# dimforge/salva

Hardware: AMD Instinct MI355X
Metric: particle-steps/sec (3D DFSPH) (higher is better)
Workload: dtype f32

## Files before the change

salva_amd/csrc/pairs.h:

```cpp
#pragma once
#include <cstdlib>

#include "tile.h"

namespace salva {

struct RecPW { float4 p, w; };
struct RecPK { float4 p; float k; };

__device__ __forceinline__ float rho0_of(const StepCtx& c, uint32_t model) {
    return (c.nmodels == 1) ? c.rho0_single : c.rho0_tab[model];
}

template <uint32_t DS>
__device__ __forceinline__ uint32_t pw_dist(const StepCtx& c, const Tile& t) { return DS ? DS * 16u : (t.stage_cap(c) + t.SB) * 16u; }
template <uint32_t DS>
__device__ __forceinline__ uint32_t pk_dist(const StepCtx& c, const Tile& t) { return DS ? DS * 16u : (t.stage_cap(c) + 2u * t.SB) * 16u; }

__device__ __forceinline__ RecPW load_pw(uint32_t o, uint32_t dist) {
    RecPW r{lds_ld16(o), lds_ld16(o + dist)};
    asm volatile("" ::"v"(r.w.w));
    return r;
}
__device__ __forceinline__ RecPK load_pk(uint32_t o, uint32_t dist) { return RecPK{lds_ld16(o), lds_ld4((o >> 2) + dist)}; }
// ... 215 lines not shown
        else if ((DSV) == FIXED_DS_LARGE) SALVA_LAUNCH_TILE_3(kernel<FIXED_DS_LARGE>, kernel<FIXED_DS_SMALL>, FIXED_DS_SMALL, kernel<0u>, c, L, lds, s, __VA_ARGS__); \
        else SALVA_LAUNCH_TILE_3(kernel<0u>, kernel<FIXED_DS_SMALL>, FIXED_DS_SMALL, kernel<0u>, c, L, lds, s, __VA_ARGS__); \
    } while (0)
static inline uint32_t pick_ds(uint32_t slots_needed, uint32_t level) {
    const uint32_t ds[3] = {FIXED_DS_SMALL, FIXED_DS_LARGE, 0u};
    uint32_t k = slots_needed <= FIXED_DS_SMALL ? 0u : (slots_needed <= FIXED_DS_LARGE ? 1u : 2u);
    k += level;
    return ds[k < 2u ? k : 2u];
}
static inline uint32_t pw_slots(const TileLds& L) { return L.sum_slots(); }
static inline uint32_t pw_bytes(const TileLds& L, uint32_t ds, bool errtab) {
    return (ds ? 2u * ds : 2u * pw_slots(L)) * 16u + (errtab ? TILE_ERR_BYTES : 0u) + 32u;
}
static inline uint32_t pick_ds_p3(uint32_t s, uint32_t level) {
    const uint32_t ds[4] = {P3_DS_THREE, P3_DS_TWO, P3_DS_ONE, 0u};
    uint32_t k = s <= P3_DS_THREE ? 0u : (s <= P3_DS_TWO ? 1u : (s <= P3_DS_ONE ? 2u : 3u));
    k += level;
    return ds[k < 3u ? k : 3u];
}
static inline uint32_t p3_bytes(const TileLds& L, uint32_t ds, uint32_t nmodels, bool with_bv) {
    const uint32_t dist8 = ds ? ds * 8u : ((L.max_halo_fluid * 8u + 15u) & ~15u);
    const uint32_t bb = with_bv ? 32u : 16u;
    const uint32_t by_maxima = ((L.max_halo_fluid * 8u + 15u) & ~15u) + bb * L.max_halo_boundary;
    const uint32_t by_raw = ((L.raw_slots() * 8u + 15u) & ~15u) + (bb - 8u) * L.max_halo_boundary;
    static const uint32_t pad = getenv("SALVA_HIP_P3_PAD") ? (uint32_t)atoi(getenv("SALVA_HIP_P3_PAD")) : 0u;
    return 2u * dist8 + (by_raw < by_maxima ? by_raw : by_maxima) + ((TILE_MAX_WAVES * nmodels * 4u + 15u) & ~15u) + 32u + pad;
}
static inline uint32_t pick_ds_p2(uint32_t n, uint32_t level) {
    const uint32_t ds[4] = {P2_DS_THREE, P3_DS_TWO, P3_DS_ONE, 0u};
    uint32_t k = n <= P2_DS_THREE ? 0u : (n <= P3_DS_TWO ? 1u : (n <= P3_DS_ONE ? 2u : 3u));
    k += level;
    return ds[k < 3u ? k : 3u];
}
#define SALVA_LAUNCH_P3(kernel, DSV, c, L, lds, s, ...)                                                                                          \
    do {                                                                                                                                         \
        if ((DSV) == P3_DS_THREE) SALVA_LAUNCH_TILE_3(kernel<P3_DS_THREE>, kernel<P3_DS_THREE>, P3_DS_THREE, kernel<0u>, c, L, lds, s, __VA_ARGS__); \
        else if ((DSV) == P3_DS_TWO) SALVA_LAUNCH_TILE_3(kernel<P3_DS_TWO>, kernel<P3_DS_THREE>, P3_DS_THREE, kernel<0u>, c, L, lds, s, __VA_ARGS__); \
        else if ((DSV) == P3_DS_ONE) SALVA_LAUNCH_TILE_3(kernel<P3_DS_ONE>, kernel<P3_DS_THREE>, P3_DS_THREE, kernel<0u>, c, L, lds, s, __VA_ARGS__); \
        else SALVA_LAUNCH_TILE_3(kernel<0u>, kernel<P3_DS_THREE>, P3_DS_THREE, kernel<0u>, c, L, lds, s, __VA_ARGS__);                             \
    } while (0)
#define SALVA_LAUNCH_P2(kernel, DSV, c, L, lds, s, ...)                                                                                          \
    do {                                                                                                                                         \
        if ((DSV) == P2_DS_THREE) SALVA_LAUNCH_TILE_3(kernel<P2_DS_THREE>, kernel<P2_DS_THREE>, P2_DS_THREE, kernel<0u>, c, L, lds, s, __VA_ARGS__); \
        else if ((DSV) == P3_DS_TWO) SALVA_LAUNCH_TILE_3(kernel<P3_DS_TWO>, kernel<P2_DS_THREE>, P2_DS_THREE, kernel<0u>, c, L, lds, s, __VA_ARGS__); \
        else if ((DSV) == P3_DS_ONE) SALVA_LAUNCH_TILE_3(kernel<P3_DS_ONE>, kernel<P2_DS_THREE>, P2_DS_THREE, kernel<0u>, c, L, lds, s, __VA_ARGS__); \
        else SALVA_LAUNCH_TILE_3(kernel<0u>, kernel<P2_DS_THREE>, P2_DS_THREE, kernel<0u>, c, L, lds, s, __VA_ARGS__);                             \
    } while (0)
static inline uint32_t pk_slots(const TileLds& L) { return L.sum_slots() + L.max_halo_boundary; }
static inline uint32_t pk_bytes(const TileLds& L, uint32_t ds) {
    return (ds ? ds : pk_slots(L)) * 16u + ((L.max_halo_fluid + 63u) & ~63u) * 4u + 32u;
}


}
```

salva_amd/csrc/switches.h:

```cpp
#pragma once
#include <cstdint>

namespace salva {

struct Switches {
    bool spec_off = true;
    bool spec_tight = false;
    bool defer_off = false;
    bool spec_apply_off = false;
    bool spec_dist_off = false;
    bool overlap_exchange = true;
    bool chain_off = false;
    bool pre_off = false;
    bool no_publish = false;
    bool split_off = false;
    uint32_t split_forced = 0;
    bool classes_off = false, classes_forced = false, light_on = false;
    bool ref_off = false, ref_forced = false;
    bool ref_tight = false;
    bool compact_halo = false;
    bool no_planes = false;
    bool no_fused_div = false;
    bool two_mass_off = false;
    uint32_t max_masses = 2;
    bool fold_off = false;
    uint32_t fold_forced = 0;
    int sort_mode = -1;
    uint32_t ds_level = 0;
    bool trust_cap0 = false;
    uint32_t list_cap0 = 0;
    bool dcs_batch_off = false;
    uint32_t dcsb_cap0 = 0;
    int field_arm = 0;
    bool tile_trace = false;
    bool dist_trace = false;
#ifdef SALVA_HIP_DIAG
    int sched_mode = 0;
    bool tile_threads_set = false;
    uint32_t tile_threads = 0;
    bool no_pipeline = false;
    uint32_t pipe_waves = 0;
    bool tile_timing = false;
#endif
    static Switches from_env();
};

}
```

salva_amd/csrc/tile.h:

```cpp
#pragma once
#include "common.h"
#include "device_types.h"

namespace salva {

#ifndef SALVA_TX
#define SALVA_TX 4
#endif
constexpr int TX = SALVA_TX, TY = 4, TZ = 4;
constexpr int TCELLS = TX * TY * TZ;
constexpr int HX = TX + 2, HY = TY + 2, HZ = TZ + 2;
constexpr int HCELLS = HX * HY * HZ;
constexpr int TILE_MAX_WAVES = 12;
constexpr int TILE_MAX_THREADS = TILE_MAX_WAVES * WAVE;

__host__ __device__ inline int floor_div(int a, int b) { return (a >= 0) ? a / b : -((-a + b - 1) / b); }

__host__ __device__ inline uint32_t ellq(uint32_t q) { return (q >> 2) * (4u * (uint32_t)WAVE) + (q & 3u); }

constexpr uint32_t TILE_TABLE_BYTES = 4 * (2 * (HCELLS + 1) + 2 * HCELLS) + 16;

struct TileLds {
    uint32_t max_halo_fluid = 0, max_halo_boundary = 0, threads = 4 * WAVE;
    uint32_t max_sum = 0;
    uint32_t max_raw = 0;
    uint32_t ds_level = 0;
    uint32_t raw_slots() const { return max_raw ? max_raw : max_halo_fluid + max_halo_boundary; }
    uint32_t sum_slots() const {
        const uint32_t worst = ((max_halo_fluid + 63u) & ~63u) + max_halo_boundary;
        return max_sum ? (max_sum < worst ? max_sum : worst) : worst;
    }
    uint32_t bytes(uint32_t bytes_per_fluid_slot, uint32_t bytes_per_boundary_slot, uint32_t narrays,
                   bool with_cell_tables = false) const {
        const uint32_t separate = ((max_halo_fluid + 63u) & ~63u) * bytes_per_fluid_slot + max_halo_boundary * bytes_per_boundary_slot;
        const uint32_t wide = bytes_per_fluid_slot > bytes_per_boundary_slot ? bytes_per_fluid_slot : bytes_per_boundary_slot;
        const uint32_t joint = sum_slots() * wide;
        return (with_cell_tables ? TILE_TABLE_BYTES : 0u) + (joint < separate ? joint : separate) + 16u * narrays;
    }
};

#ifndef SALVA_FIXED_DS_SMALL
#define SALVA_FIXED_DS_SMALL 2448
#endif
constexpr uint32_t FIXED_DS_SMALL = SALVA_FIXED_DS_SMALL, FIXED_DS_LARGE = 3984;
#ifndef SALVA_P3_DS3
#define SALVA_P3_DS3 2080
#endif
constexpr uint32_t P3_DS_THREE = SALVA_P3_DS3, P3_DS_TWO = 3360, P3_DS_ONE = 4064;
#ifndef SALVA_P2_DS3
#define SALVA_P2_DS3 2464
#endif
constexpr uint32_t P2_DS_THREE = SALVA_P2_DS3;
static_assert((P3_DS_THREE % 64 == 32 && P3_DS_TWO % 64 == 32 && P3_DS_ONE % 64 == 32 && P2_DS_THREE % 64 == 32) || SALVA_P3_DS3 != 2080 || SALVA_P2_DS3 != 2464,
              "plane distances: odd multiples of 256 bytes");
constexpr uint32_t TILE_PART_SHIFT = 28;
constexpr uint32_t TILE_PART_WHOLE = (uint32_t)(TX - 1) << 2;
// ... 943 lines not shown
```

salva_amd/csrc/world.h:

```cpp
#pragma once
#include <functional>
#include <string>
#include <map>
#include <memory>
#include <vector>

#include "../../include/salva_hip.h"
#include "common.h"
#include "device_types.h"
#include "comm.h"
#include "dist.h"
#include "kernels.h"
#include "elastic.h"
#include "switches.h"
#include "mesh.h"
#include "compound.h"
#include "sink.h"
#include "field.h"
#include "anisotropy.h"
#include "surface.h"
#include "fluidcast.h"

namespace salva {

// ... 407 lines not shown
        GridShape gs;
        double dcs_ms = 0.0;
        int attempt = 0;
        bool dcs_undo = false;
        uint32_t split_s_cur = 0;
        bool two_mass = false;
        uint32_t nmass = 0; float mass_classes[4] = {0.0f, 0.0f, 0.0f, 0.0f}; uint64_t mass_cmask = 0;
        size_t dist_ev_used = 0; std::vector<std::pair<size_t, int>> dist_ev_pairs;
    } pass;
    struct GridTabs;
    struct PassSnapshot;
    void prepare_working_set(SalvaHipStepStats& st);
    GridShape choose_grid();
    void ensure_slot_tables(uint32_t nslots_bound);
    bool run_pass(const PassSnapshot& snap, float& dt, const float g[3], SalvaHipStepStats& st);
    void enqueue_grid_keys(GridTabs& T, const GridShape& gs, bool counting, bool mass, const uint32_t* gate);
    void enqueue_grid_sort(GridTabs& T, const GridShape& gs, bool counting, const uint32_t* gate);
    size_t tile_scan_temp(const GridShape& gs);
    uint32_t enqueue_grid_tiles(GridTabs& T, const GridShape& gs, StepCtx c, size_t tb, const uint32_t* gate, bool publish);
    bool predict_totals(const GridShape& gs, TileAcc& tt) const;
    void reorder_working_set(bool timers);
    void size_pass(uint32_t seq_totals);
    void fill_tile_tables(bool again);
    void build_lists();
    void density_and_solve(StepCtx& c, float& dt, const float g[3], SalvaHipStepStats& st, bool timers);
    void publish_end_of_step(const PassSnapshot& snap);
    void adopt_chain_outcome(StepCtx& c, float& dt, const float g[3], SalvaHipStepStats& st, bool timers);
    int finish_substep(float dt, SalvaHipStepStats& st);
    void record_timers(SalvaHipStepStats& st);
    void raise_step_flags();
    bool has_force(int kind) const;
    bool counting_sort_for(size_t ncf, uint32_t np) const;
    void grow_list_caps(uint32_t need_ff, uint32_t need_fb);
    int cfl_mode = 0;
    float cfl_coeff = 0.4f;
    int cfl_min_sub = 1, cfl_max_sub = 10;
    float step_total = 0.0f, step_remaining = 0.0f;
    std::vector<float> substeps;
    float choose_substep(const StepCtx& c);
    FluidArrays arrays(int which);
    DistArrays dist_arrays(int which);
    void dist_prepare();
    void dist_build_lists();
    template <typename T, typename Gather, typename Scatter> void refresh_ghosts(T* field, Gather gather, Scatter scatter);
    void refresh_f32(float* field);
    void refresh_f4(float4* field);
    void ensure_particle_capacity(size_t cap);
    void allreduce_host_u64(std::vector<unsigned long long>& v);
    uint32_t num_models() const { return (uint32_t)std::max<size_t>(fluids.size(), 1); }
    template <typename Decide> void allreduced_test(const SolveCtl* record, Decide&& decide);
    void finalize_solve(SolveCtl* ctl, SolveCtl* pub, uint32_t skipped);
    void finalize_solve_ring(int it, SolveCtl* pub);

    const Switches sw = Switches::from_env();
    uint32_t last_iters[NUM_SOLVES] = {1u, 1u, 1u};
    uint32_t prev_iters[NUM_SOLVES] = {1u, 1u, 1u};
    float mass_uniform = 0.0f;
    bool mass_known = false;
    bool flags_clean = false;
    bool lists_checked = false;
    uint32_t fold_relax = 0;
    bool fold_locked = false;
    bool split_on = false;
    int32_t bbox_used_last[6] = {0, 0, 0, 0, 0, 0}; bool bbox_used_valid = false;
    TileAcc pred_tt{};
    uint32_t pred_n = 0; bool pred_valid = false;
    bool ref_pred_valid = false;
    uint32_t ref_pred[3] = {0, 0, 0}, ref_pred_n = 0;
    bool ref_last = false;
    RefCaps ref_last_caps{0xffffffffu, 0xffffffffu, 0xffffffffu};
    TileLds lds_full;
    uint32_t ref_last_nslots_bound = 0;
    struct Tallies { uint64_t chain_steps = 0, chain_breaks = 0, spec_misses = 0, ref_passes = 0, ref_misses = 0, pre_adopted = 0, pre_dropped = 0; } tally;

    hipStream_t stream = nullptr;
    hipStream_t stream2 = nullptr;
    hipStream_t dl_stream = nullptr;
    hipEvent_t ev_dl_ready = nullptr, ev_dl_done = nullptr;
    DevBuf<float> dl_dev[2];
    float* h_dl[2] = {nullptr, nullptr};
    size_t h_dl_cap[2] = {0, 0};
    struct PendingDownload { bool active = false; float* dst[2] = {nullptr, nullptr}; bool staged[2] = {false, false}; size_t bytes = 0; } dl;
    hipEvent_t ev_pre_refresh = nullptr, ev_interior = nullptr;
    hipEvent_t ev_spec_eval = nullptr, ev_spec_apply = nullptr;
    template <typename Launch> void evaluate_split(const StepCtx& c, int iteration, Launch&& launch);
    uint32_t n = 0, nb = 0;

    DevBuf<float4> st_pos, st_vel, st_dv, st_acc;
    DevBuf<uint32_t> st_model;
    bool staging_current = true, sorted_valid = false, acc_user = false;

    DevBuf<float4> posm[2], vel[2], dv[2];
    DevBuf<uint32_t> model[2], perm[2];
// ... 136 lines not shown
```

salva_amd/csrc/world.hip:

```cpp
#include "world.h"
#include "bbox.h"

#include <algorithm>
#include <cmath>
#include <cstring>
#include <limits>

#include <mutex>
#include <unordered_map>

namespace salva {

void raise_tile_lds_limit(const void* kernel, uint32_t bytes) {
    if (bytes > 160u * 1024u)
        throw HipError(SALVA_HIP_E_CAPACITY, "a tile's halo does not fit the 160 KiB LDS (particles are compressed far beyond rest density)");
    static std::mutex mu;
    static std::unordered_map<const void*, uint32_t> granted;
    std::lock_guard<std::mutex> lock(mu);
    uint32_t& g = granted[kernel];
    if (bytes <= g) return;
    const uint32_t want = std::min<uint32_t>(160u * 1024u, std::max<uint32_t>(bytes + bytes / 4, 64u * 1024u));
    SALVA_HIP_CHECK(hipFuncSetAttribute(kernel, hipFuncAttributeMaxDynamicSharedMemorySize, (int)want));
    g = want;
}
// ... 10 lines not shown
    s.spec_dist_off = on("SALVA_HIP_NO_SPEC_DIST");
    s.overlap_exchange = !on("SALVA_HIP_NO_OVERLAP");
    s.spec_off = !on("SALVA_HIP_SPECULATE") || on("SALVA_HIP_NO_SPECULATION");
    s.spec_tight = on("SALVA_HIP_SPEC_TIGHT");
    s.defer_off = on("SALVA_HIP_NO_DEFER_LISTS");
    s.spec_apply_off = on("SALVA_HIP_NO_SPEC_APPLY");
    s.chain_off = on("SALVA_HIP_NO_CHAIN");
    s.pre_off = on("SALVA_HIP_NO_PREGRID");
    s.no_publish = on("SALVA_HIP_NO_PUBLISH");
    s.split_off = on("SALVA_HIP_NO_SPLIT");
    s.classes_off = on("SALVA_HIP_NO_CLASSES");
    s.classes_forced = on("SALVA_HIP_CLASSES");
    s.light_on = on("SALVA_HIP_LIGHT");
    s.ref_off = on("SALVA_HIP_FULL_HALO");
    s.ref_forced = on("SALVA_HIP_REF_HALO");
    s.ref_tight = on("SALVA_HIP_REF_TIGHT");
    s.compact_halo = on("SALVA_HIP_COMPACT_HALO");
    if (const char* e = getenv("SALVA_HIP_SPLIT_S")) s.split_forced = (uint32_t)std::max(atoi(e), 1);
    s.no_planes = on("SALVA_HIP_NO_PLANES");
    s.two_mass_off = on("SALVA_HIP_NO_TWO_MASS");
    if (const char* e = getenv("SALVA_HIP_MAX_MASSES")) s.max_masses = (uint32_t)std::min(std::max(atoi(e), 2), 4);
    s.fold_off = on("SALVA_HIP_NO_FOLD");
    if (const char* e = getenv("SALVA_HIP_FOLD_CELLS")) {
        const long v = atol(e);
        if (v >= 8 && v <= (1 << 20) && (v & (v - 1)) == 0) s.fold_forced = (uint32_t)v;
    }
    s.tile_trace = on("SALVA_HIP_TILE_TRACE");
    s.dist_trace = on("SALVA_HIP_DIST_TRACE");
    s.no_fused_div = on("SALVA_HIP_NO_FUSED_DIV");
    s.dcs_batch_off = on("SALVA_HIP_NO_DCS_BATCH");
    if (const char* e = getenv("SALVA_HIP_FIELD_ARM")) s.field_arm = !strcmp(e, "points") ? 1 : !strcmp(e, "lattice") ? 2 : 0;
    if (const char* e = getenv("SALVA_HIP_DCSB_CAP0")) s.dcsb_cap0 = (uint32_t)std::max(atoi(e), 1);
    if (const char* e = getenv("SALVA_HIP_RADIX_SORT")) s.sort_mode = atoi(e) != 0 ? 1 : 0;
    if (const char* e = getenv("SALVA_HIP_DS_LEVEL")) s.ds_level = (uint32_t)std::max(0, atoi(e));
    if (const char* e = getenv("SALVA_HIP_LIST_CAP0")) { s.list_cap0 = std::max<uint32_t>(LIST_REGS, ((uint32_t)atoi(e) + 3u) & ~3u); s.trust_cap0 = true; }
#ifdef SALVA_HIP_DIAG
    if (const char* e = getenv("SALVA_HIP_SCHED")) s.sched_mode = atoi(e);
    if (const char* e = getenv("SALVA_HIP_TILE_THREADS")) { s.tile_threads = (uint32_t)atoi(e); s.tile_threads_set = true; }
    s.no_pipeline = on("SALVA_HIP_NO_PIPELINE");
    if (const char* e = getenv("SALVA_HIP_PIPE_WAVES")) s.pipe_waves = std::min<uint32_t>(std::max(atoi(e), 1), PIPE_MAX_WAVES);
    s.tile_timing = on("SALVA_HIP_TILE_TIMING");
#endif
    return s;
}

World::World(const SalvaHipParams& p) : prm(p) {
    if (!(p.particle_radius > 0.0f) || !(p.smoothing_factor > 0.0f))
        throw HipError(SALVA_HIP_E_INVALID, "particle_radius and smoothing_factor must be positive");
    if (p.solver != SALVA_HIP_SOLVER_DFSPH && p.solver != SALVA_HIP_SOLVER_IISPH)
        throw HipError(SALVA_HIP_E_INVALID, "unknown solver kind");
    int ndev = 0;
    hipError_t e = hipGetDeviceCount(&ndev);
    if (e != hipSuccess || ndev == 0)
        throw HipError(SALVA_HIP_E_HIP, "no HIP device available: libsalva_hip has no CPU fallback");
    if (p.device < 0 || p.device >= ndev) throw HipError(SALVA_HIP_E_INVALID, "device ordinal out of range");
    use_device();
    const float h = p.particle_radius * p.smoothing_factor * 2.0f;
    sc = make_sph_consts(h);
    if (p.kernel_density < 0 || p.kernel_density > SALVA_HIP_KERNEL_VISCOSITY || p.kernel_gradient < 0 || p.kernel_gradient > SALVA_HIP_KERNEL_VISCOSITY)
        throw HipError(SALVA_HIP_E_INVALID, "unknown kernel kind");
    sc.kd = p.kernel_density;
    sc.kg = p.kernel_gradient;
    SALVA_HIP_CHECK(hipStreamCreateWithFlags(&stream, hipStreamNonBlocking));
    SALVA_HIP_CHECK(hipStreamCreateWithFlags(&stream2, hipStreamNonBlocking));
    SALVA_HIP_CHECK(hipEventCreateWithFlags(&ev_pre_refresh, hipEventDisableTiming));
    SALVA_HIP_CHECK(hipEventCreateWithFlags(&ev_interior, hipEventDisableTiming));
// ... 56 lines not shown
    for (uint32_t s = 0; s < slot; ++s) o += fluids[s].n;
    return o;
}
uint64_t World::boundary_offset(uint32_t slot) const {
    uint64_t o = 0;
    for (uint32_t s = 0; s < slot; ++s) o += bounds[s].n;
    return o;
}
World::SlotSpan World::fluid_span(uint32_t slot) const {
    if (slot >= fluids.size()) throw HipError(SALVA_HIP_E_INVALID, "fluid slot out of range");
    return {fluids[slot].n, fluid_offset(slot)};
}
World::SlotSpan World::boundary_span(uint32_t slot) const {
    if (slot >= bounds.size()) throw HipError(SALVA_HIP_E_INVALID, "boundary slot out of range");
    return {bounds[slot].n, boundary_offset(slot)};
}

FluidArrays World::arrays(int which) {
    FluidArrays a;
    a.posm = posm[which].p; a.vel = vel[which].p; a.dv = dv[which].p; a.model = model[which].p; a.perm = perm[which].p;
    a.gtag = comm ? gtag[which].p : nullptr;
    return a;
}

void World::ensure_cub_temp(size_t bytes) { cub_temp.ensure(bytes ? bytes : 1, stream, false, 1.25f); }

static inline bool groups_test(uint32_t m1, uint32_t f1, uint32_t m2, uint32_t f2) {
    return (m1 & f2) != 0 && (m2 & f1) != 0;
}

void World::upload_tables() {
    if (!tables_dirty) return;
    lists_checked = sw.trust_cap0;
    const uint32_t nm = num_models(), nbm = (uint32_t)std::max<size_t>(bounds.size(), 1);
    std::vector<float> r0(nm, 1000.0f);
    std::vector<uint32_t> counts(nm, 0);
    std::vector<uint8_t> ff(nm * nm, 1), fb(nm * nbm, 1), bb(nbm * nbm, 1), bw(nbm, 0);
    any_wants_forces = false;
    for (uint32_t a = 0; a < fluids.size(); ++a) {
        r0[a] = fluids[a].density0;
        counts[a] = (uint32_t)fluids[a].n;
        for (uint32_t b = 0; b < fluids.size(); ++b)
            ff[a * nm + b] = (a == b) || groups_test(fluids[a].memberships, fluids[a].filter, fluids[b].memberships, fluids[b].filter);
        for (uint32_t b = 0; b < bounds.size(); ++b)
            fb[a * nbm + b] = groups_test(fluids[a].memberships, fluids[a].filter, bounds[b].memberships, bounds[b].filter);
    }
    for (uint32_t a = 0; a < bounds.size(); ++a) {
        bw[a] = bounds[a].wants_forces ? 1 : 0;
        any_wants_forces |= bounds[a].wants_forces;
        for (uint32_t b = 0; b < bounds.size(); ++b)
            bb[a * nbm + b] = (a == b) || groups_test(bounds[a].memberships, bounds[a].filter, bounds[b].memberships, bounds[b].filter);
    }
    rho0_tab.ensure(nm); model_counts.ensure(nm); ff_ok.ensure(nm * nm); fb_ok.ensure(nm * nbm); bb_ok.ensure(nbm * nbm); bwants.ensure(nbm);
    SALVA_HIP_CHECK(hipMemcpyAsync(rho0_tab.p, r0.data(), nm * sizeof(float), hipMemcpyHostToDevice, stream));
    if (comm && dist_started && global_counts.size() == nm) counts = global_counts;
    SALVA_HIP_CHECK(hipMemcpyAsync(model_counts.p, counts.data(), nm * sizeof(uint32_t), hipMemcpyHostToDevice, stream));
    SALVA_HIP_CHECK(hipMemcpyAsync(ff_ok.p, ff.data(), ff.size(), hipMemcpyHostToDevice, stream));
    SALVA_HIP_CHECK(hipMemcpyAsync(fb_ok.p, fb.data(), fb.size(), hipMemcpyHostToDevice, stream));
    SALVA_HIP_CHECK(hipMemcpyAsync(bb_ok.p, bb.data(), bb.size(), hipMemcpyHostToDevice, stream));
    SALVA_HIP_CHECK(hipMemcpyAsync(bwants.p, bw.data(), bw.size(), hipMemcpyHostToDevice, stream));
    SALVA_HIP_CHECK(hipStreamSynchronize(stream));
    tables_dirty = false;
    b_dirty = true;
}

float World::bforce_scale() const {
// ... 182 lines not shown
    add(bforce.bytes()); add(bperm.bytes()); add(cell_start_b.bytes()); add(partials.bytes());
    return b;
}

template <typename Launch>
static float time_launches(hipStream_t stream, hipEvent_t begin, hipEvent_t end, int reps, Launch&& launch) {
    launch();
    SALVA_HIP_CHECK(hipEventRecord(begin, stream));
    for (int r = 0; r < reps; ++r) launch();
    SALVA_HIP_CHECK(hipEventRecord(end, stream));
    SALVA_HIP_CHECK(hipStreamSynchronize(stream));
    float ms = 0.0f;
    SALVA_HIP_CHECK(hipEventElapsedTime(&ms, begin, end));
    return ms * 1000.0f / (float)reps;
}

void World::tile_tables(uint32_t slot, uint32_t* info, uint32_t* halo_row, uint32_t cap_row, uint32_t* counts, uint32_t cap_counts, uint32_t* entries,
                        uint32_t cap_entries) {
    use_device();
    if (!have_last_ctx || !sorted_valid || n == 0) throw HipError(SALVA_HIP_E_INVALID, "no completed step to look at");
    const StepCtx& c = last_ctx;
    if (slot >= c.nlaunch) throw HipError(SALVA_HIP_E_INVALID, "no such tile slot");
    SALVA_HIP_CHECK(hipStreamSynchronize(stream));
    TileAcc a[2];
    uint4 desc;
    SALVA_HIP_CHECK(hipMemcpy(a, c.tile_off + slot, sizeof(a), hipMemcpyDeviceToHost));
    SALVA_HIP_CHECK(hipMemcpy(&desc, c.slot_desc + slot, sizeof(desc), hipMemcpyDeviceToHost));
    const uint32_t S = (uint32_t)(a[1].s - a[0].s), SB = (uint32_t)(a[1].sb - a[0].sb), own_n = desc.z - desc.y;
    const uint64_t hoff = c.halo_stride ? (uint64_t)slot * c.halo_stride : a[0].s;
    memset(info, 0, 16 * sizeof(uint32_t));
    info[0] = c.nlaunch; info[1] = desc.y; info[2] = desc.z; info[3] = S; info[4] = SB;
    info[5] = lds.max_halo_fluid; info[6] = lds.raw_slots(); info[7] = lds.sum_slots(); info[8] = lds_full.max_halo_fluid;
    info[9] = ref_last ? 1u : 0u; info[10] = (uint32_t)tally.ref_passes; info[11] = (uint32_t)tally.ref_misses;
    if (halo_row && cap_row && S)
        SALVA_HIP_CHECK(hipMemcpy(halo_row, c.halo_src + hoff, (size_t)std::min(S, cap_row) * sizeof(uint32_t), hipMemcpyDeviceToHost));
    if (!own_n) return;
    std::vector<uint32_t> cnt(own_n);
    SALVA_HIP_CHECK(hipMemcpy(cnt.data(), c.nff + desc.y, (size_t)own_n * sizeof(uint32_t), hipMemcpyDeviceToHost));
    if (counts) memcpy(counts, cnt.data(), (size_t)std::min(own_n, cap_counts) * sizeof(uint32_t));
    if (!entries || !cap_entries) return;
    const uint32_t nsl = (own_n + WAVE - 1) / WAVE;
    std::vector<uint32_t> blk((size_t)nsl * c.cap_ff * WAVE);
    SALVA_HIP_CHECK(hipMemcpy(blk.data(), c.nbr_ff + (size_t)a[0].nsl * c.cap_ff * WAVE, blk.size() * sizeof(uint32_t), hipMemcpyDeviceToHost));
    uint32_t o = 0;
    for (uint32_t k = 0; k < own_n; ++k) {
        const uint32_t* p = blk.data() + (size_t)(k / WAVE) * c.cap_ff * WAVE + 4u * (k % WAVE);
        for (uint32_t e = 0; e < cnt[k] && o < cap_entries; ++e) {
            const uint32_t d = p[ellq(e >> 1)];
            entries[o++] = (e & 1u) ? (d >> 16) : (d & 0xffffu);
        }
    }
    info[12] = o;
}

float World::time_kernel(int kernel, int reps) {
    use_device();
    if (!have_last_ctx || !sorted_valid || n == 0) throw HipError(SALVA_HIP_E_INVALID, "no completed step to time");
    if (reps < 1) reps = 1;
#ifdef SALVA_HIP_DIAG
    if (kernel == 0 && sw.tile_timing) tile_timing_report();
#endif
    const bool iisph = prm.solver == SALVA_HIP_SOLVER_IISPH;
    if (kernel == 4 && comm) throw HipError(SALVA_HIP_E_INVALID, "not available in a multi-GPU run");
    if ((kernel == 2 || kernel == 3) && !iisph) throw HipError(SALVA_HIP_E_INVALID, "an IISPH kernel needs an IISPH world");
    if (kernel == 1 && iisph) throw HipError(SALVA_HIP_E_INVALID, "k_divergence needs a DFSPH world");
    StepCtx cd = last_ctx;
// ... 74 lines not shown
```

salva_amd/csrc/world_step.hip:

```cpp
#include "world.h"
#include "bbox.h"

#include <algorithm>
#include <cfloat>
#include <cstddef>
#include <chrono>
#include <cmath>
#include <cstring>
#include <limits>

namespace salva {

__global__ void k_bforce_fold(uint32_t nb, unsigned long long* __restrict__ fx, float4* __restrict__ bforce, float inv_scale) {
    const uint32_t i = blockIdx.x * blockDim.x + threadIdx.x;
    if (i >= nb) return;
    unsigned long long* f = fx + 3ull * i;
    float4 b = bforce[i];
    b.x += (float)((double)(long long)f[0] * (double)inv_scale);
    b.y += (float)((double)(long long)f[1] * (double)inv_scale);
    b.z += (float)((double)(long long)f[2] * (double)inv_scale);
    bforce[i] = b;
    f[0] = f[1] = f[2] = 0ull;
}

// ... 626 lines not shown
struct World::PassSnapshot {
    int32_t bbox[6];
    float dt_prev, inv_dt_prev;
    int cur;
    uint32_t last_iters[NUM_SOLVES], prev_iters[NUM_SOLVES];
    explicit PassSnapshot(const World& w) : dt_prev(w.dt_prev), inv_dt_prev(w.inv_dt_prev), cur(w.cur) {
        memcpy(bbox, w.h_rb->bbox, sizeof(bbox));
        memcpy(last_iters, w.last_iters, sizeof(last_iters));
        memcpy(prev_iters, w.prev_iters, sizeof(prev_iters));
    }
    void restore(World& w) const {
        w.cur = cur; w.dt_prev = dt_prev; w.inv_dt_prev = inv_dt_prev;
        memcpy(w.h_rb->bbox, bbox, sizeof(bbox));
        memcpy(w.last_iters, last_iters, sizeof(last_iters)); memcpy(w.prev_iters, prev_iters, sizeof(prev_iters));
        if (w.pre.valid) { w.pre.valid = false; w.pre_drop(); }
    }
};

bool World::has_force(int kind) const {
    for (const FluidSlot& f : fluids)
        for (const SalvaHipForceDesc& d : f.forces)
            if (d.kind == kind) return true;
    return false;
}

bool World::counting_sort_for(size_t ncf, uint32_t n) const {
    return ncf + 1 < 0x7fffffffull && (sw.sort_mode == 0 || (sw.sort_mode < 0 && ncf <= 16ull * n + (1ull << 20)));
}

void World::grow_list_caps(uint32_t need_ff, uint32_t need_fb) {
    if (need_ff > cap_ff) cap_ff = (need_ff + need_ff / 4 + 4u) & ~3u;
    if (need_fb > cap_fb) cap_fb = (need_fb + need_fb / 4 + 4u) & ~3u;
}

static bool halo_fits(const TileAcc& tt, uint32_t max_sum) {
    TileLds probe; probe.max_halo_fluid = tt.max_s; probe.max_halo_boundary = tt.max_sb; probe.max_sum = max_sum;
    return tt.max_s < 65536u && tt.max_sb < 65536u && probe.bytes(52, 32, 6) <= 160u * 1024u;
}

void World::enqueue_grid_keys(GridTabs& T, const GridShape& gs, bool counting, bool mass, const uint32_t* gate) {
    const uint32_t nslots = std::max<uint32_t>(gs.nslots_bound, 1u);
    T.cell_start_f.ensure(gs.ncf + 1, stream, false, 1.5f);
    T.tile_flags.ensure((size_t)gs.ntiles + 1, stream, false, 1.5f);
    T.tile_rank.ensure((size_t)gs.ntiles + 1, stream, false, 1.5f);
    T.tile_ids.ensure(nslots, stream, false, 1.5f);
    T.slot_desc.ensure(nslots, stream, false, 1.5f);
    T.tile_cnt.ensure((size_t)gs.nslots_bound + 1, stream, false, 1.5f);
    T.tile_off.ensure((size_t)gs.nslots_bound + 1, stream, false, 1.5f);
    if (counting) {
        T.cell_rank.ensure(n, stream, false, 1.1f);
        SALVA_HIP_CHECK(hipMemsetAsync(T.cell_start_f.p, 0, (gs.ncf + 1) * sizeof(uint32_t), stream));
    }
    launch_cell_keys(posm[cur].p, n, sc.h, gf.device(nullptr), T.keys[0].p, T.idx[0].p, d_flags.p, mass ? mass_slots.p : nullptr,
                     counting ? T.cell_start_f.p : nullptr, counting ? T.cell_rank.p : nullptr, stream, gate);
}
void World::enqueue_grid_sort(GridTabs& T, const GridShape& gs, bool counting, const uint32_t* gate) {
    if (counting) {
        const size_t tb = cell_sort_temp_bytes((uint32_t)gs.ncf);
        ensure_cub_temp(tb);
        cell_sort(cub_temp.p, tb, n, (uint32_t)gs.ncf, T.keys[0].p, T.cell_rank.p, T.cell_start_f.p, T.keys[1].p, T.idx[0].p, T.idx[1].p, stream, gate);
    } else {
        const int end_bit = bits_for(gs.ncf);
        const size_t tb = sort_pairs_temp_bytes(n, end_bit);
        ensure_cub_temp(tb);
        sort_pairs(cub_temp.p, tb, T.keys[0].p, T.keys[1].p, T.idx[0].p, T.idx[1].p, n, end_bit, stream);
        launch_cell_start(T.keys[1].p, n, (uint32_t)gs.ncf, T.cell_start_f.p, stream);
// ... 141 lines not shown
            memcpy(&m, &h_rb->mass_mm[0], sizeof(m));
            mass_uniform = (h_rb->mass_mm[0] == h_rb->mass_mm[1] && m > 0.0f && std::isfinite(m) && !sw.no_planes) ? m : 0.0f;
            mass_known = true;
        }
    }
    p.nlaunch = tt.nonempty;
    lds.max_halo_fluid = tt.max_s; lds.max_halo_boundary = tt.max_sb;
    lds.max_sum = spec ? 0u : tt.max_sum;
    lds.max_raw = spec ? 0u : tt.max_raw;
    if (sw.tile_trace)
        fprintf(stderr, "salva_hip tiles: nonempty %u max_s %u max_sb %u max_sum %u max_raw %u heavy %u light %u tiny %u split_s %u mass_uniform %g | chained %llu breaks %llu pregrid %llu dropped %llu | fold %u %u %u\n",
                tt.nonempty, tt.max_s, tt.max_sb, tt.max_sum, tt.max_raw, tt.heavy, tt.nlight, tt.ntiny, p.split_s_cur, (double)mass_uniform,
                (unsigned long long)tally.chain_steps, (unsigned long long)tally.chain_breaks, (unsigned long long)tally.pre_adopted, (unsigned long long)tally.pre_dropped,
                gf.mask[0] + 1u, gf.mask[1] + 1u, gf.mask[2] + 1u);
    if (!spec) {
        if (!split_on) split_on = tt.heavy > 0u && (uint64_t)tt.heavy * 5u <= tt.nonempty;
        else if ((uint64_t)tt.heavy * 2u > tt.nonempty) split_on = false;
    }
#ifndef SALVA_TILE_WAVES_CAP
#define SALVA_TILE_WAVES_CAP 8
#endif
    static_assert(SALVA_TILE_WAVES_CAP <= TILE_MAX_WAVES, "the launch bounds are written for TILE_MAX_WAVES");
    const uint32_t avg = (n + tt.nonempty - 1) / std::max<uint32_t>(tt.nonempty, 1u);
    const uint32_t lo = (HCELLS + WAVE - 1) / WAVE, hi = std::min<uint32_t>(std::max<uint32_t>(tt.max_nsl, lo), (uint32_t)(SALVA_TILE_WAVES_CAP));
#ifdef SALVA_TILE_WAVES_PLAIN_AVERAGE
    const uint32_t weighted = 0u;
#else
    const uint32_t weighted = tt.nsl ? (uint32_t)((double)tt.wsl / (double)tt.nsl + 0.5) : 0u;
#endif
    lds.threads = WAVE * std::min<uint32_t>(std::max<uint32_t>(std::max<uint32_t>((avg + WAVE - 1) / WAVE, weighted), lo), hi);
#ifdef SALVA_HIP_DIAG
    if (sw.tile_threads_set) lds.threads = sw.tile_threads;
#endif
    if (gf.folded() && !fold_locked && !spec && !halo_fits(tt, tt.max_sum)) {
        ++fold_relax;
        throw FoldRetry{};
    }
    if (lds.max_halo_fluid >= 65536u || lds.max_halo_boundary >= 65536u)
        throw HipError(SALVA_HIP_E_CAPACITY, "more than 65535 particles in one tile halo");
    if (tt.nsl > n / WAVE + p.gs.nslots_bound + 1) throw HipError(SALVA_HIP_E_HIP, "internal error: slice count exceeds its bound");
    const uint64_t st_f = (lds.max_halo_fluid + 63u) & ~63u, st_b = nb ? ((lds.max_halo_boundary + 63u) & ~63u) : 0u;
    const uint64_t strided = (uint64_t)p.nlaunch * (st_f + st_b), compact = tt.s + tt.sb;
    const bool use = strided <= 3 * compact + (1u << 20) && !sw.compact_halo;
    halo_stride = use ? (uint32_t)st_f : 0u; bhalo_stride = use ? (uint32_t)st_b : 0u;
#ifdef SALVA_HIP_DIAG
    pipe.enabled = halo_stride > 0 && !sw.no_pipeline;
    pipe.scap = halo_stride; pipe.sbcap = bhalo_stride;
    pipe.num_cus = (uint32_t)num_cus; pipe.nlaunch = p.nlaunch;
    uint32_t waves = std::min<uint32_t>(std::max<uint32_t>(tt.max_nsl, 4u), (uint32_t)PIPE_MAX_WAVES);
    if (sw.pipe_waves) waves = sw.pipe_waves;
    pipe.threads = waves * WAVE;
#endif
    p.need_f = halo_stride ? (size_t)p.nlaunch * halo_stride : (size_t)tt.s;
    p.need_b = halo_stride ? (size_t)p.nlaunch * bhalo_stride : (size_t)tt.sb;
    halo_src.ensure(p.need_f ? p.need_f : 1, stream, false, 1.2f);
    bhalo_src.ensure(p.need_b ? p.need_b : 1, stream, false, 1.2f);
    p.nslices = tt.nsl;
    if (spec) {
        p.spec_mode = true;
        p.halo_cap = lds.max_halo_fluid; p.bhalo_cap = lds.max_halo_boundary; p.nslices_cap = p.nslices;
        p.halo_len = p.need_f; p.bhalo_len = p.need_b;
    }
    const bool beyond3 = tt.max_s > P3_DS_THREE || tt.max_raw > P2_DS_THREE || tt.max_sum > FIXED_DS_SMALL;
    if (!spec && !sw.classes_off) {
        if (tt.ntiny > 0u && tt.ntiny < tt.nonempty && (sw.classes_forced || tt.ntiny >= 512u)) p.class_ntiny = tt.ntiny;
        const uint32_t nfull = tt.nonempty - tt.nlight - tt.ntiny;
// ... 3 lines not shown
    if (p.class_ntiny || p.class_nlight) slot_order.ensure(p.nlaunch, stream, false, 1.5f);
    if (p.class_nlight) ++counters.light_class_passes;
    if (p.class_ntiny) ++counters.sparse_class_passes;

    p.ref_step = !sw.ref_off && !spec && n > 0 && halo_stride > 0u && p.c.nmodels <= 32u && p.c.nbmodels <= 32u && (sw.ref_forced || beyond3);
    p.refb = RefBuild{halo_src.p, slot_info.p, G().tile_off.p, RefCaps{0xffffffffu, 0xffffffffu, 0xffffffffu}, d_rb.p->max_ref};
    if (p.ref_step && p.defer_lists && ref_pred_valid && ref_pred_n == n) {
        auto bound = [&](uint32_t pred, uint32_t full, uint32_t layout) {
            if (sw.ref_tight) return std::min(pred - pred / 8u, full);
            uint32_t b = pred + std::max<uint32_t>(96u, pred / 8u);
            if (b > layout && pred + 8u <= layout) b = layout;
            return std::min(b, full);
        };
        p.refb.cap.s = bound(ref_pred[0], tt.max_s, P3_DS_THREE);
        p.refb.cap.raw = std::max(bound(ref_pred[1], tt.max_raw, P2_DS_THREE), tt.max_sb);
        p.refb.cap.sum = std::max(bound(ref_pred[2], tt.max_sum, FIXED_DS_SMALL), tt.max_sb);
        p.ref_bounded = true;
    }
}

void World::fill_tile_tables(bool again) {
    const Pass& p = pass;
    StepCtx c = make_ctx();
    c.slot_order = nullptr; c.ntiny = c.nlight = 0u;
    if (again) scan_tiles(cub_temp.p, p.scan_tb, G().tile_cnt.p, G().tile_off.p, p.gs.nslots_bound + 1, stream);
    launch_tile_halo_fill(c, halo_src.p, bhalo_src.p, slot_info.p, stream, (p.class_ntiny || p.class_nlight) ? slot_order.p : nullptr, p.class_nlight, p.class_ntiny);
}

void World::build_lists() {
    Pass& p = pass;
    fill_tile_tables(false);
    for (int nattempt = 0;; ++nattempt) {
        if (nattempt > 0 && p.ref_step) fill_tile_tables(true);
        nbr_ff.ensure((size_t)p.nslices * cap_ff * WAVE + 1, stream, false, 1.1f);
        nbr_fb.ensure(nb ? (size_t)p.nslices * cap_fb * WAVE + 1 : 1, stream, false, 1.1f);
        slice_near.ensure((size_t)p.nslices + 1, stream, false, 1.1f);
        p.c = make_ctx();
        p.fold_stats = (p.spec || p.defer_lists) && n > 0;
        launch_nbr_build(p.c, lds, tile_list_stats.p, p.fold_stats ? nullptr : reinterpret_cast<unsigned long long*>(&d_rb.p->ncontacts_ff),
                         &d_rb.p->max_cnt_ff, comm ? reinterpret_cast<unsigned long long*>(&d_rb.p->ncontacts_own_ff) : nullptr, stream,
                         p.ref_step ? &p.refb : nullptr);
        if (p.spec || p.defer_lists) break;
        static_assert(offsetof(Readback, max_cnt_ff) == offsetof(Readback, ncontacts_ff) + 2 * sizeof(uint64_t), "list statistics travel in one copy");
        publish_and_wait(nullptr, true, false);
        const uint32_t need_ff = (h_rb->max_cnt_ff + 1) / 2, need_fb = (h_rb->max_cnt_fb + 1) / 2;
        if (need_ff <= cap_ff && need_fb <= cap_fb) break;
        if (nattempt >= 2) throw HipError(SALVA_HIP_E_HIP, "internal error: neighbour list capacity did not converge");
        grow_list_caps(need_ff, need_fb);
    }
    lds_full = lds; ref_last = p.ref_step; ref_last_caps = p.refb.cap; ref_last_nslots_bound = p.gs.nslots_bound;
    if (p.ref_step) {
        if (!p.defer_lists) { lds.max_halo_fluid = std::max<uint32_t>(h_rb->max_ref[0], 1u); lds.max_raw = h_rb->max_ref[1]; lds.max_sum = h_rb->max_ref[2]; }
        else if (p.ref_bounded) { lds.max_halo_fluid = p.refb.cap.s; lds.max_raw = p.refb.cap.raw; lds.max_sum = p.refb.cap.sum; }
        p.ref_on_cur = true;
        ++tally.ref_passes;
        if (sw.tile_trace && !p.defer_lists)
            fprintf(stderr, "salva_hip halo: full max_s %u max_raw %u | referenced max_s %u max_raw %u max_sum %u | staged bound %u (exact)\n",
                    p.tt.max_s, p.tt.max_raw, h_rb->max_ref[0], h_rb->max_ref[1], h_rb->max_ref[2], lds.max_halo_fluid);
    }
#ifdef SALVA_HIP_DIAG
    if (sw.sched_mode > 0) launch_list_schedule(p.c, lds, stream);
#endif
}

void World::density_and_solve(StepCtx& c, float& dt, const float g[3], SalvaHipStepStats& st, bool timers) {
    pass.fused_first_divergence = prm.solver == SALVA_HIP_SOLVER_DFSPH && !sw.no_fused_div && launch_density_alpha_div(c, lds, stream);
    pass.iisph_dii_fused = prm.solver == SALVA_HIP_SOLVER_IISPH && !comm && !sw.no_fused_div && !cfl_mode;
// ... 91 lines not shown
    if (p.timers) SALVA_HIP_CHECK(hipEventRecord(ev[2], stream));
    publish_end_of_step(snap);
    if (comm && prm.enable_timers) dist_time_fold();

    const uint32_t need_ff = (h_rb->max_cnt_ff + 1) / 2, need_fb = (h_rb->max_cnt_fb + 1) / 2;
    bool miss = false;
    if (p.defer_lists && !p.spec) {
        const bool ref_miss = p.ref_bounded && (h_rb->flags & 16u) != 0u;
        if (ref_miss) { ref_pred_valid = false; ++tally.ref_misses; }
        if (p.ref_on_cur && sw.tile_trace)
            fprintf(stderr, "salva_hip halo: full max_s %u max_raw %u | referenced max_s %u max_raw %u max_sum %u | staged bound %u (%s)%s\n",
                    lds_full.max_halo_fluid, lds_full.max_raw, h_rb->max_ref[0], h_rb->max_ref[1], h_rb->max_ref[2], lds.max_halo_fluid,
                    p.ref_bounded ? "previous step + margin" : "full box", ref_miss ? " MISS: pass repeated" : "");
        miss = need_ff > cap_ff || need_fb > cap_fb || ref_miss;
    }
    if (p.spec) {
        const TileAcc& a = h_rb->tile_total;
        miss = !(a.nonempty <= p.tt.nonempty && a.max_s <= p.tt.max_s && a.max_sb <= p.tt.max_sb && a.nsl <= p.tt.nsl &&
                 (halo_stride || (a.s <= p.tt.s && a.sb <= p.tt.sb)) && need_ff <= cap_ff && need_fb <= cap_fb);
        if (miss) ++tally.spec_misses;
        ++counters.speculative_passes;
    }
    if (miss) {
        ++counters.discarded_passes;
        snap.restore(*this);
        grow_list_caps(need_ff, need_fb);
        return false;
    }
    if (p.chain_pending) adopt_chain_outcome(p.c, dt, g, st, p.timers);
    pred_tt = h_rb->tile_total; pred_n = n; pred_valid = true;
    if (p.ref_on_cur) { memcpy(ref_pred, h_rb->max_ref, sizeof(ref_pred)); ref_pred_n = n; ref_pred_valid = true; }
    else ref_pred_valid = false;
    lists_checked = true;
    return true;
}

void World::record_timers(SalvaHipStepStats& st) {
    const Pass& p = pass;
    const double untimed = std::numeric_limits<double>::quiet_NaN();
    bool ok = hipEventSynchronize(ev[2]) == hipSuccess;
    if (!ok) (void)hipGetLastError();
    auto ms = [&](hipEvent_t from, hipEvent_t to) -> double {
        float t = 0.0f;
        if (!ok) return untimed;
        if (hipEventElapsedTime(&t, from, to) != hipSuccess) { (void)hipGetLastError(); return untimed; }
        return (double)t;
    };
    const double a = ms(ev[0], ev[1]), b = ms(ev[1], ev[2]);
    st.grid_ms += (float)a; st.solver_ms += (float)b; st.step_ms += (float)(a + b);
    counters.step_time += a + b;
    counters.stages.collision_detection_time += a;
    counters.stages.solver_time += b;
    counters.cd.boundary_update_time += p.dcs_ms;
    const double gi = ms(ev[0], evc[1]);
    counters.cd.grid_insertion_time += std::isnan(gi) ? gi : std::max(0.0, gi - p.dcs_ms);
    counters.cd.neighborhood_search_time += ms(evc[1], ev[1]);
    counters.solver.pressure_resolution_time += ms(evc[2], ev[2]);
    if (prm.solver == SALVA_HIP_SOLVER_DFSPH) counters.custom += ms(evc[3], evc[4]);
}

void World::raise_step_flags() {
    static const struct { uint32_t bit; int code; const char* what; } fatal[] = {
        {1u, SALVA_HIP_E_NUMERIC, "zero density / boundary denominator or NaN detected (the reference would panic)"},
        {2u, SALVA_HIP_E_HIP, "internal error: particle outside the cell table"},
        {8u, SALVA_HIP_E_HIP, "internal error: a third particle mass in a world the host took for a two-mass world"},
        {16u, SALVA_HIP_E_HIP, "internal error: a referenced halo beyond its bound in a pass that had none"}};
// ... 70 lines not shown
```

Baseline: 408.2 million.

## Grow neighbour list capacities ahead of demand and add apply-wave thread override

After a successful list check, neighbour-list capacities are raised predictively from the recent rise in required counts, and power-of-two capacities are padded. The aim is to avoid discarded speculative passes and rebuilds when list demand creeps up. The ff list buffer also gets a larger growth slack factor. An env-controlled thread count for P2 launches is added, off by default. The cost is more memory and slightly longer neighbour-list strides.

```diff
diff --git a/salva_amd/csrc/pairs.h b/salva_amd/csrc/pairs.h
--- a/salva_amd/csrc/pairs.h
+++ b/salva_amd/csrc/pairs.h
@@ -271,15 +271,22 @@
     k += level;
     return ds[k < 3u ? k : 3u];
 }
-#define SALVA_LAUNCH_P3(kernel, DSV, c, L, lds, s, ...)                                                                                          \
+#define SALVA_LAUNCH_P3(kernel, DSV, c, L, lds, s, ...)                                                                                         \
     do {                                                                                                                                         \
         if ((DSV) == P3_DS_THREE) SALVA_LAUNCH_TILE_3(kernel<P3_DS_THREE>, kernel<P3_DS_THREE>, P3_DS_THREE, kernel<0u>, c, L, lds, s, __VA_ARGS__); \
         else if ((DSV) == P3_DS_TWO) SALVA_LAUNCH_TILE_3(kernel<P3_DS_TWO>, kernel<P3_DS_THREE>, P3_DS_THREE, kernel<0u>, c, L, lds, s, __VA_ARGS__); \
         else if ((DSV) == P3_DS_ONE) SALVA_LAUNCH_TILE_3(kernel<P3_DS_ONE>, kernel<P3_DS_THREE>, P3_DS_THREE, kernel<0u>, c, L, lds, s, __VA_ARGS__); \
         else SALVA_LAUNCH_TILE_3(kernel<0u>, kernel<P3_DS_THREE>, P3_DS_THREE, kernel<0u>, c, L, lds, s, __VA_ARGS__);                             \
     } while (0)
+static inline TileLds p2_launch_lds(const TileLds& L) {
+    TileLds t = L;
+    if (t.threads_apply) t.threads = t.threads_apply;
+    return t;
+}
 #define SALVA_LAUNCH_P2(kernel, DSV, c, L, lds, s, ...)                                                                                          \
     do {                                                                                                                                         \
+        const ::salva::TileLds _lp2 = ::salva::p2_launch_lds(L);                                                                                 \
+        const ::salva::TileLds L = _lp2;                                                                                                         \
         if ((DSV) == P2_DS_THREE) SALVA_LAUNCH_TILE_3(kernel<P2_DS_THREE>, kernel<P2_DS_THREE>, P2_DS_THREE, kernel<0u>, c, L, lds, s, __VA_ARGS__); \
         else if ((DSV) == P3_DS_TWO) SALVA_LAUNCH_TILE_3(kernel<P3_DS_TWO>, kernel<P2_DS_THREE>, P2_DS_THREE, kernel<0u>, c, L, lds, s, __VA_ARGS__); \
         else if ((DSV) == P3_DS_ONE) SALVA_LAUNCH_TILE_3(kernel<P3_DS_ONE>, kernel<P2_DS_THREE>, P2_DS_THREE, kernel<0u>, c, L, lds, s, __VA_ARGS__); \
diff --git a/salva_amd/csrc/switches.h b/salva_amd/csrc/switches.h
--- a/salva_amd/csrc/switches.h
+++ b/salva_amd/csrc/switches.h
@@ -26,6 +26,7 @@
     bool fold_off = false;
     uint32_t fold_forced = 0;
     int sort_mode = -1;
+    uint32_t apply_waves = 0;
     uint32_t ds_level = 0;
     bool trust_cap0 = false;
     uint32_t list_cap0 = 0;
diff --git a/salva_amd/csrc/tile.h b/salva_amd/csrc/tile.h
--- a/salva_amd/csrc/tile.h
+++ b/salva_amd/csrc/tile.h
@@ -22,6 +22,7 @@
 
 struct TileLds {
     uint32_t max_halo_fluid = 0, max_halo_boundary = 0, threads = 4 * WAVE;
+    uint32_t threads_apply = 0;
     uint32_t max_sum = 0;
     uint32_t max_raw = 0;
     uint32_t ds_level = 0;
diff --git a/salva_amd/csrc/world.h b/salva_amd/csrc/world.h
--- a/salva_amd/csrc/world.h
+++ b/salva_amd/csrc/world.h
@@ -463,6 +463,7 @@
     bool has_force(int kind) const;
     bool counting_sort_for(size_t ncf, uint32_t np) const;
     void grow_list_caps(uint32_t need_ff, uint32_t need_fb);
+    void grow_caps_ahead(uint32_t need_ff, uint32_t need_fb);
     int cfl_mode = 0;
     float cfl_coeff = 0.4f;
     int cfl_min_sub = 1, cfl_max_sub = 10;
@@ -490,6 +491,7 @@
     bool mass_known = false;
     bool flags_clean = false;
     bool lists_checked = false;
+    uint32_t need_last[2] = {0, 0}; bool need_last_valid = false;
     uint32_t fold_relax = 0;
     bool fold_locked = false;
     bool split_on = false;
diff --git a/salva_amd/csrc/world.hip b/salva_amd/csrc/world.hip
--- a/salva_amd/csrc/world.hip
+++ b/salva_amd/csrc/world.hip
@@ -66,6 +66,7 @@
     if (const char* e = getenv("SALVA_HIP_FIELD_ARM")) s.field_arm = !strcmp(e, "points") ? 1 : !strcmp(e, "lattice") ? 2 : 0;
     if (const char* e = getenv("SALVA_HIP_DCSB_CAP0")) s.dcsb_cap0 = (uint32_t)std::max(atoi(e), 1);
     if (const char* e = getenv("SALVA_HIP_RADIX_SORT")) s.sort_mode = atoi(e) != 0 ? 1 : 0;
+    if (const char* e = getenv("SALVA_HIP_APPLY_WAVES")) s.apply_waves = (uint32_t)std::min(std::max(atoi(e), 4), TILE_MAX_WAVES);
     if (const char* e = getenv("SALVA_HIP_DS_LEVEL")) s.ds_level = (uint32_t)std::max(0, atoi(e));
     if (const char* e = getenv("SALVA_HIP_LIST_CAP0")) { s.list_cap0 = std::max<uint32_t>(LIST_REGS, ((uint32_t)atoi(e) + 3u) & ~3u); s.trust_cap0 = true; }
 #ifdef SALVA_HIP_DIAG
@@ -188,6 +189,7 @@
 void World::upload_tables() {
     if (!tables_dirty) return;
     lists_checked = sw.trust_cap0;
+    need_last_valid = false;
     const uint32_t nm = num_models(), nbm = (uint32_t)std::max<size_t>(bounds.size(), 1);
     std::vector<float> r0(nm, 1000.0f);
     std::vector<uint32_t> counts(nm, 0);
@@ -436,6 +438,7 @@
     info[0] = c.nlaunch; info[1] = desc.y; info[2] = desc.z; info[3] = S; info[4] = SB;
     info[5] = lds.max_halo_fluid; info[6] = lds.raw_slots(); info[7] = lds.sum_slots(); info[8] = lds_full.max_halo_fluid;
     info[9] = ref_last ? 1u : 0u; info[10] = (uint32_t)tally.ref_passes; info[11] = (uint32_t)tally.ref_misses;
+    info[13] = lds.threads; info[14] = lds.threads_apply ? lds.threads_apply : lds.threads; info[15] = cap_ff;
     if (halo_row && cap_row && S)
         SALVA_HIP_CHECK(hipMemcpy(halo_row, c.halo_src + hoff, (size_t)std::min(S, cap_row) * sizeof(uint32_t), hipMemcpyDeviceToHost));
     if (!own_n) return;
diff --git a/salva_amd/csrc/world_step.hip b/salva_amd/csrc/world_step.hip
--- a/salva_amd/csrc/world_step.hip
+++ b/salva_amd/csrc/world_step.hip
@@ -682,6 +682,21 @@
     if (need_ff > cap_ff) cap_ff = (need_ff + need_ff / 4 + 4u) & ~3u;
     if (need_fb > cap_fb) cap_fb = (need_fb + need_fb / 4 + 4u) & ~3u;
 }
+void World::grow_caps_ahead(uint32_t need_ff, uint32_t need_fb) {
+    const uint32_t need[2] = {need_ff, need_fb};
+    uint32_t* const cap[2] = {&cap_ff, &cap_fb};
+    for (int k = 0; k < (nb ? 2 : 1); ++k) {
+        const uint32_t rise = (need_last_valid && need[k] > need_last[k]) ? need[k] - need_last[k] : 0u;
+        const uint32_t ahead = need[k] + std::max<uint32_t>(rise, 1u);
+        if (ahead > *cap[k]) {
+            uint32_t c = (ahead + 3u) & ~3u;
+            if ((c & (c - 1u)) == 0u) c += 4u;
+            *cap[k] = c;
+        }
+        need_last[k] = need[k];
+    }
+    need_last_valid = true;
+}
 
 static bool halo_fits(const TileAcc& tt, uint32_t max_sum) {
     TileLds probe; probe.max_halo_fluid = tt.max_s; probe.max_halo_boundary = tt.max_sb; probe.max_sum = max_sum;
@@ -889,6 +904,7 @@
 #ifdef SALVA_HIP_DIAG
     if (sw.tile_threads_set) lds.threads = sw.tile_threads;
 #endif
+    lds.threads_apply = sw.apply_waves ? sw.apply_waves * WAVE : 0u;
     if (gf.folded() && !fold_locked && !spec && !halo_fits(tt, tt.max_sum)) {
         ++fold_relax;
         throw FoldRetry{};
@@ -958,7 +974,7 @@
     fill_tile_tables(false);
     for (int nattempt = 0;; ++nattempt) {
         if (nattempt > 0 && p.ref_step) fill_tile_tables(true);
-        nbr_ff.ensure((size_t)p.nslices * cap_ff * WAVE + 1, stream, false, 1.1f);
+        nbr_ff.ensure((size_t)p.nslices * cap_ff * WAVE + 1, stream, false, 1.2f);
         nbr_fb.ensure(nb ? (size_t)p.nslices * cap_fb * WAVE + 1 : 1, stream, false, 1.1f);
         slice_near.ensure((size_t)p.nslices + 1, stream, false, 1.1f);
         p.c = make_ctx();
@@ -1116,6 +1132,7 @@
     if (p.ref_on_cur) { memcpy(ref_pred, h_rb->max_ref, sizeof(ref_pred)); ref_pred_n = n; ref_pred_valid = true; }
     else ref_pred_valid = false;
     lists_checked = true;
+    grow_caps_ahead(need_ff, need_fb);
     return true;
 }
 
```

Measured after the change: 413.4 million (median of 6 runs). 1.01x the previous value.
